# qiyueyao/Kubernetes-verification

Hardware: AMD Instinct MI355X
Metric: pod-pairs/sec for reachability build + all-checks latency, 100k pods, 1/2/4/8 GPU (higher is better)
Workload: dtype u64

## Files before the change

### include/kano_hip.h

```cpp
#ifndef KANO_HIP_H
#define KANO_HIP_H

#include <stddef.h>
#include <stdint.h>

#ifdef __cplusplus
extern "C" {
#endif

typedef struct kano_ctx kano_ctx;

#define KANO_PATH_AUTO    0
#define KANO_PATH_BITWISE 1
#define KANO_PATH_MFMA    2

#define KANO_INFO_N        0
#define KANO_INFO_W        1
#define KANO_INFO_P        2
#define KANO_INFO_U        3
#define KANO_INFO_NNZ_SEL  4
#define KANO_INFO_NNZ_ALW  5
#define KANO_INFO_HEAVY    6
#define KANO_INFO_ROW0     7
#define KANO_INFO_ROW1     8
#define KANO_INFO_MAXSEL   9
#define KANO_INFO_UA      10
#define KANO_INFO_HEAVY_PATH 11
#define KANO_INFO_WORK_ITEMS 12
#define KANO_INFO_ROWS_KERNEL 13
#define KANO_INFO_ROWS_CUS 14
#define KANO_INFO_HEAVY_SEL 15
#define KANO_INFO_HEAVY_KERNEL 16
#define KANO_INFO_CLS_REUSED 17
#define KANO_INFO_NSLOTS   18

int  kano_create(int device, kano_ctx** out);
int  kano_create_lean(int device, kano_ctx** out);
void kano_destroy(kano_ctx* ctx);
const char* kano_last_error(const kano_ctx* ctx);
int  kano_set_stream(kano_ctx* ctx, void* hip_stream);

int kano_set_pods(kano_ctx* ctx, int64_t n, int32_t ncols, const int32_t* pod_val);
int kano_set_policies(kano_ctx* ctx, int64_t P,
                      const int64_t* sel_off, const int32_t* sel_col, const int32_t* sel_val,
                      const int64_t* alw_off, const int32_t* alw_col, const int32_t* alw_val);
int kano_set_shard(kano_ctx* ctx, int64_t row_begin, int64_t row_end);

int kano_build(kano_ctx* ctx, int path);
int kano_info(kano_ctx* ctx, int64_t* out );

int kano_col_checks(kano_ctx* ctx, uint64_t* col_and, uint64_t* col_or);
int kano_col_flags_dev(kano_ctx* ctx, uint8_t* flags_dev);

int kano_crosscheck(kano_ctx* ctx, const int32_t* gid, uint64_t* cross);
int kano_crosscheck_dev(kano_ctx* ctx, const int32_t* gid, uint8_t* flags_dev);

int kano_get_rows(kano_ctx* ctx, int64_t r0, int64_t nrows, uint64_t* dst);
// ... 205 lines not shown
```

### kubernetes-verification_amd/csrc/kano_engine.hpp

```cpp
#pragma once
#include <hip/hip_runtime.h>
#include <hip/hip_ext.h>

#include <algorithm>
#include <cmath>
#include <functional>
#include <cerrno>
#include <cstdint>
#include <cstdlib>
#include <cstring>
#include <string>
#include <vector>
#include <array>
#include <chrono>
#include <ctime>
#include <cstdio>
#include <dlfcn.h>
#include <link.h>
#include <thread>

#include "kano_hip.h"
#include "kano_internal.hpp"
#include "kano_pairwalk.hpp"
#include "kano_prims.hpp"
// ... 115 lines not shown
  int group_grid = 0;
  int group_batches = 0;
  int shadow_r = 0;
  int shg_sub_lds = 1;
  int rows_cu_off = 20;
  int xcd_split = 1;
  i64 xcd_min_bytes = XCD_MIN_BYTES;
  int xcd_write = XCD_WRITE;
  int xcd_eng0 = -1;
  bool xcd_tried = false, eng_on_xcd = false, xcd_last_ok = false;
  int side_mode = 0;
  int xcd_side = -1;
  hipStream_t stream_x = nullptr, stream2_x = nullptr, stream3x = nullptr;
  hipStream_t stream2_u = nullptr;
  hipEvent_t ev_sw = nullptr, ev_sw2 = nullptr;
  i64 rows_cu_bytes = 8ll << 30;
  int num_cus = 0, rows_cus = 0;

  ClassSet rc, cc;
  bool cls_valid = false;
  bool cls_reuse = false;
  i64 cls_U[2] = {0, 0};
  i64 cls_reused = 0;
  SideMatch sm, am;
  i64 UAW = 0, ldC = 0;
  i64 nnz_sel = 0, nnz_alc = 0, nnz_alw = 0, heavy_count = 0, wi_total = 0, nflags = 0;
  i64 heavy_sel = 0;
  i64 light_cost = 0;
  bool rows_use_alist = false;
  int max_sel = 0;
  int heavy_path = 0;
  int heavy_kernel = 0;
  int rows_kernel = 0;

  DBuf pv;
  DBuf scnt, cost, soffc, scur, slist, ecls, wicls, maxs, wicnt, wioff, hflag, hoff, hlist, sq, pfoff;
  DBuf ACT, AC, nca, acnt, alcoff, alc, aloff, alist;
  DBuf M, Mc, color, colnand, col_and, col_or_c, col_nand_c;
  DBuf scan_tmp;
  i64 scan_cap = 0;
  int scan_parity = 0;
  DBuf scan_tmp2;
  i64 scan_cap2 = 0;
  int scan_parity2 = 0;
  hipEvent_t ev_pre = nullptr, ev_pre_done = nullptr, ev_pre_ac = nullptr;
  bool pre_forked = false, pre_side_pending = false, pre_ac_pending = false;
// ... 202 lines not shown
```

### kubernetes-verification_amd/csrc/kano_hip.hip

```cpp
#include "kano_engine.hpp"
#include "kano_kernels.hpp"

namespace kano_eng {

int fail(kano_ctx* ctx, int code, const std::string& msg) {
  ctx->err = msg;
  return code;
}

int settle(kano_ctx* ctx);

int dalloc(kano_ctx* ctx, DBuf& b, size_t bytes) {
  if (bytes == 0) bytes = 16;
  if (b.p && b.bytes >= bytes) return 0;
  if (b.p) {
    KTRY(settle(ctx));
    KCHK(hipFree(b.p));
    b.p = nullptr;
    b.bytes = 0;
  }
  const hipError_t e = hipMalloc(&b.p, bytes);
  if (e != hipSuccess) {
    b.p = nullptr;
    return fail(ctx, -ENOMEM, "hipMalloc(" + std::to_string(bytes) + " bytes) -> " +
// ... 1062 lines not shown
  if (ctx->pre_side_pending) {
    ctx->pre_side_pending = false;
    KTRY(join_event(ctx, ctx->ev_pre_done));
  }
  ctx->alist_valid = false;
  ctx->rows_use_alist = ctx->light_cost > 0 && ctx->light_cost * 16 > ctx->nnz_alw &&
                        ctx->nnz_alw * 4 <= (2ll << 30);
  const McScatterArgs msa{ctx->nnz_sel, P_<int32_t>(ctx->ecls), P_<int32_t>(ctx->slist),
                          P_<i64>(ctx->alcoff), P_<int32_t>(ctx->alc), P_<int32_t>(ctx->rc.mcnt),
                          H > 0 ? P_<int32_t>(ctx->hflag) : (const int32_t*)nullptr,
                          P_<u64>(ctx->Mc), ldMc};
  const bool scatter_on = U > 0 && ctx->nnz_sel > 0;
  const bool pods_in_scatter = ctx->rows_use_alist && scatter_on && P > 0 && ctx->cc.U > 0;
  if (ctx->rows_use_alist) KTRY(build_alist(ctx, nullptr, !pods_in_scatter));
  ctx->rin_marked = false;
  if (U == 0) return ctx->fork_hook ? ctx->fork_hook(fork_marked) : 0;
  hipEvent_t rin_mark = H == 0 && ctx->cols_deferred ? ctx->ev_rin_e : nullptr;
  if (scatter_on && (size_t)ldMc * 8 * (TPB / 64) <= 64 * 1024) {
    const size_t lds = sizeof(u64) * (size_t)ldMc * (TPB / 64);
    const McOwnArgs moa{U, P_<i64>(ctx->soffc), P_<int32_t>(ctx->slist), P_<i64>(ctx->alcoff),
                        P_<int32_t>(ctx->alc), P_<int32_t>(ctx->rc.mcnt),
                        H > 0 ? P_<int32_t>(ctx->hflag) : (const int32_t*)nullptr,
                        P_<u64>(ctx->Mc), ldMc};
    if (pods_in_scatter) {
      const unsigned nb1 = nblk(P, WPB);
      hipExtLaunchKernelGGL(k_pods_own, dim3(nb1 + nblk(U, TPB / 64)), dim3(TPB), lds,
                            ctx->stream, nullptr, rin_mark, 0, pol_pods_args(ctx), moa, nb1);
    } else {
      hipExtLaunchKernelGGL(k_mc_own, dim3(nblk(U, TPB / 64)), dim3(TPB), lds, ctx->stream,
                            nullptr, rin_mark, 0, moa);
    }
    KLAUNCH();
    ctx->rin_marked = rin_mark != nullptr;
  } else if (scatter_on) {
    if (pods_in_scatter) {
      const unsigned nb1 = nblk(P, WPB);
      hipExtLaunchKernelGGL(k_pods_scatter, dim3(nb1 + nblk(ctx->nnz_sel, TPB / 64)), dim3(TPB),
                            0, ctx->stream, nullptr, rin_mark, 0, pol_pods_args(ctx), msa, nb1);
    } else {
      hipExtLaunchKernelGGL(k_mc_scatter, dim3(nblk(ctx->nnz_sel, TPB / 64)), dim3(TPB), 0,
                            ctx->stream, nullptr, rin_mark, 0, msa);
    }
    KLAUNCH();
    ctx->rin_marked = rin_mark != nullptr;
  }
  if (H > 0) {
    if (mfma) {
// ... 82 lines not shown
    } else {
      if (ctx->time_or) {
        KTRY(resolve_mfma_time(ctx));
        KCHK(hipEventRecord(ctx->ev_m0, ctx->stream));
      }
      hipLaunchKernelGGL(k_heavy_mc_or, dim3((unsigned)H, nblk(ldMc, 64)), dim3(TPB), 0, ctx->stream,
                         P_<int32_t>(ctx->hlist), P_<i64>(ctx->soffc), P_<int32_t>(ctx->slist),
                         P_<u64>(ctx->AC), ctx->ldC, ctx->UAW, P_<u64>(ctx->Mc), ldMc);
      KLAUNCH();
      if (ctx->time_or) {
        KCHK(hipEventRecord(ctx->ev_m1, ctx->stream));
        ctx->mfma_time_pending = true;
        ctx->mfma_ops_last = 2.0 * (double)H * (double)P * (double)ctx->cc.U;
      }
    }
    const bool early = ctx->rows_early_heavy == 1 ||
                       (ctx->rows_early_heavy == 2 &&
                        std::min<i64>(ctx->ldM, ctx->rows_cww) > 4096);
    if (early && ctx->cols_deferred && !ctx->rin_marked) {
      KCHK(hipEventRecord(ctx->ev_rin_e, ctx->stream));
      ctx->rin_marked = true;
    }
  }
  if (!ctx->cols_deferred) KTRY(mc_cols(ctx));
  if (ctx->fork_hook) KTRY(ctx->fork_hook(fork_marked));
  return 0;
}

int do_rows(kano_ctx* ctx) {
  const i64 ldM = ctx->ldM, n = ctx->n;
  if (n > 0) {
    hipLaunchKernelGGL(k_cols_expand, dim3(nblk(ldM * 64)), dim3(TPB), 0, ctx->stream,
                       P_<u64>(ctx->col_or_c), P_<u64>(ctx->col_nand_c), P_<int32_t>(ctx->cc.cls),
                       n, ldM, P_<u64>(ctx->color), P_<u64>(ctx->colnand));
    KLAUNCH();
  } else {
    KCHK(hipMemsetAsync(ctx->color.p, 0, sizeof(u64) * ldM, ctx->stream));
    KCHK(hipMemsetAsync(ctx->colnand.p, 0, sizeof(u64) * ldM, ctx->stream));
  }
  return 0;
}

thread_local bool g_create_lean = false;
void rows_cu_mask(int K, uint32_t* mask) {
  const int t = K < 4 ? 1 : K / 4, beta = K < 4 ? K : 4;
  for (int w = 0; w < 8; ++w) {
    mask[w] = 0xffffffffu;
// ... 296 lines not shown
  int32_t G = ngroups;
  cp.gdev = P_<int32_t>(ctx->gid);
  if (!gid) {
    if (ctx->groups_n != n) return fail(ctx, -EINVAL, "crosscheck: no stored groups for these pods");
    G = ctx->groups_G;
    cp.gdev = P_<int32_t>(ctx->gids);
  } else {
    if (G <= 0) {
      G = 0;
      for (i64 i = 0; i < n; ++i) {
        if (gid[i] < 0) return fail(ctx, -EINVAL, "kano_crosscheck: negative group id");
        G = std::max(G, gid[i] + 1);
      }
    }
    KCHK(hipMemcpyAsync(ctx->gid.p, gid, sizeof(int32_t) * n, hipMemcpyHostToDevice,
                        st ? st : ctx->stream));
  }
  cp.G = G;
  cp.on = true;
  return 0;
}

int cross_prepare(kano_ctx* ctx, const int32_t* gid, int32_t ngroups, CrossPlan& cp,
                  FillBatch& fb, bool setup_done = false) {
  const i64 ldM = ctx->ldM;
  if (!setup_done) KTRY(cross_setup(ctx, gid, ngroups, cp, fb.st));
  int32_t* err = reinterpret_cast<int32_t*>(P_<u64>(ctx->sizes) + SZ_ERR);
  KTRY(fb.add_raw(err, sizeof(u64), 0u));
  KTRY(fb.add(ctx->cross, sizeof(u64) * ldM, 0u));
  if (!cp.on) return 0;
  const int32_t G = cp.G;
  if (ctx->rows_dirty) return 0;
  const i64 U = ctx->rc.U, ldC = ctx->ldC;
  KTRY(dalloc(ctx, ctx->gmin, sizeof(int32_t) * std::max<i64>(1, U)));
  KTRY(dalloc(ctx, ctx->gmax, sizeof(int32_t) * std::max<i64>(1, U)));
  KTRY(dalloc(ctx, ctx->R, sizeof(u64) * std::max<i64>(1, (i64)G * ldC)));
  KTRY(dalloc(ctx, ctx->ckey, sizeof(int32_t) * std::max<i64>(1, U)));
  KTRY(dalloc(ctx, ctx->corder, sizeof(int32_t) * std::max<i64>(1, U)));
  cp.key_lds = (i64)G + 1 <= KEY_LDS_MAX;
  cp.knb = std::max<i64>(1, nblk(U, (i64)TPB * KEY_ITEMS));
  cp.kslots = cp.key_lds ? ((i64)G + 1) * cp.knb : (i64)G + 1;
  KTRY(dalloc(ctx, ctx->kcnt, sizeof(int32_t) * 2 * ((i64)G + 1) + sizeof(int32_t) * cp.kslots));
  KTRY(dalloc(ctx, ctx->koff, sizeof(int32_t) * (cp.kslots + 1)));
  KTRY(dalloc(ctx, ctx->multi, sizeof(u64) * ldC));
  KTRY(dalloc(ctx, ctx->A1, sizeof(u64) * ldC));
  KTRY(dalloc(ctx, ctx->A2, sizeof(u64) * ldC));
  KTRY(fb.add(ctx->gmin, sizeof(int32_t) * U, 0x7fffffffu));
  KTRY(fb.add(ctx->gmax, sizeof(int32_t) * U, 0xffffffffu));
  KTRY(fb.add(ctx->R, sizeof(u64) * (i64)G * ldC, 0u));
  for (DBuf* b : {&ctx->multi, &ctx->A1, &ctx->A2}) KTRY(fb.add(*b, sizeof(u64) * ldC, 0u));
  KTRY(fb.add(ctx->kcnt, sizeof(int32_t) * 2 * ((i64)G + 1), 0u));
  return 0;
}

KeySort cross_sort(kano_ctx* ctx, const CrossPlan& cp) {
  KeySort k{};
  k.U = ctx->rc.U;
  k.nb = cp.knb;
  k.mcnt = P_<int32_t>(ctx->rc.mcnt);
  k.gmin = P_<int32_t>(ctx->gmin);
  k.gmax = P_<int32_t>(ctx->gmax);
  k.G = cp.G;
  k.ckey = P_<int32_t>(ctx->ckey);
  k.hist = P_<int32_t>(ctx->kcnt) + 2 * ((i64)cp.G + 1);
  k.hoff = P_<int32_t>(ctx->koff);
  k.order = P_<int32_t>(ctx->corder);
  return k;
}

int cross_stage_a(kano_ctx* ctx, const CrossPlan& cp, ScanBatch& sb, hipStream_t st = nullptr) {
  if (!cp.on) return 0;
  const i64 U = ctx->rc.U, G = cp.G, rl = rows_local(ctx);
  const hipStream_t s = st ? st : ctx->stream;
  int32_t* err = reinterpret_cast<int32_t*>(P_<u64>(ctx->sizes) + SZ_ERR);
  hipLaunchKernelGGL(k_cls_group_range_m, dim3(nblk(rl)), dim3(TPB), 0, s, cp.gdev,
                     (int32_t)G, P_<int32_t>(ctx->rc.cls), P_<int32_t>(ctx->rc.mem), rl,
                     P_<int32_t>(ctx->gmin), P_<int32_t>(ctx->gmax), err);
  KLAUNCH();
  int32_t* kcnt = P_<int32_t>(ctx->kcnt);
  if (cp.key_lds) {
    const KeySort ks = cross_sort(ctx, cp);
    hipLaunchKernelGGL(k_key_hist, dim3((unsigned)cp.knb), dim3(TPB),
                       sizeof(int32_t) * (size_t)(G + 1), s, ks);
    KLAUNCH();
    if (!st) KTRY(sb.add(ks.hist, cp.kslots, P_<int32_t>(ctx->koff)));
  } else {
    hipLaunchKernelGGL(k_cls_key, dim3(nblk(U)), dim3(TPB), 0, s, U,
                       P_<int32_t>(ctx->rc.mcnt), P_<int32_t>(ctx->gmin), P_<int32_t>(ctx->gmax),
                       (int32_t)G, P_<int32_t>(ctx->ckey), kcnt);
    KLAUNCH();
    KTRY(sb.add(kcnt, G + 1, P_<int32_t>(ctx->koff)));
  }
  return 0;
}

int cross_stage_b1(kano_ctx* ctx, const CrossPlan& cp, hipStream_t st = nullptr) {
  if (!cp.on) return 0;
  const i64 U = ctx->rc.U, G = cp.G;
  const hipStream_t s = st ? st : ctx->stream;
  int32_t* kcnt = P_<int32_t>(ctx->kcnt);
  if (cp.key_lds && st) {
    hipLaunchKernelGGL(k_key_place_scan, dim3((unsigned)cp.knb), dim3(TPB),
                       sizeof(int32_t) * (size_t)(G + 1), s, cross_sort(ctx, cp));
  } else if (cp.key_lds) {
    hipLaunchKernelGGL(k_key_place_lds, dim3((unsigned)cp.knb), dim3(TPB),
                       sizeof(int32_t) * (size_t)(G + 1), s, cross_sort(ctx, cp));
  } else {
    hipLaunchKernelGGL(k_cls_key_place, dim3(nblk(U)), dim3(TPB), 0, s, U,
                       P_<int32_t>(ctx->ckey), P_<int32_t>(ctx->koff), kcnt + G + 1,
                       P_<int32_t>(ctx->corder));
  }
  KLAUNCH();
  return 0;
}

int cross_stage_b2(kano_ctx* ctx, const CrossPlan& cp) {
  if (!cp.on) return 0;
  const i64 U = ctx->rc.U, G = cp.G, ldC = ctx->ldC, UAW = ctx->UAW;
  const bool cols = ctx->cols_deferred;
  const int32_t* nlive = P_<int32_t>(ctx->koff) + cp.kslots;
  {
    const int32_t* ord = P_<int32_t>(ctx->corder);
    const int32_t* ck = P_<int32_t>(ctx->ckey);
    u64* co = cols ? P_<u64>(ctx->col_or_c) : nullptr;
    u64* cn = cols ? P_<u64>(ctx->col_nand_c) : nullptr;
    const dim3 g(nblk(UAW, 64), nblk(U, (TPB / 64) * FOLD_PER_WAVE));
    hipLaunchKernelGGL(k_mc_fold, g, dim3(TPB), 0, ctx->stream, P_<u64>(ctx->Mc), ldC, UAW,
                       ctx->cc.U, ord, nlive, ck, (int32_t)G, P_<u64>(ctx->R),
                       P_<u64>(ctx->multi), co, cn);
  }
  KLAUNCH();
  ctx->cols_deferred = false;
  hipLaunchKernelGGL(k_cross_groups, dim3((unsigned)G, nblk(UAW)), dim3(TPB), 0, ctx->stream,
                     P_<u64>(ctx->R), ldC, UAW, P_<u64>(ctx->A1), P_<u64>(ctx->A2));
  KLAUNCH();
  ctx->cross_G = (int32_t)G;
  return 0;
}

int crosscheck_impl(kano_ctx* ctx, const int32_t* gid, int32_t ngroups = 0) {
  const i64 n = ctx->n, W = ctx->W, ldM = ctx->ldM;
  CrossPlan cp;
  {
    FillBatch fb(ctx);
// ... 276 lines not shown
        if (k == "pmf" && v >= 0 && v <= 2) ctx->pmask_form = v;
        if (k == "pmgrid" && v >= 0) ctx->pmask_grid = v;
        if (k == "pvf" && v >= 0 && v <= 2) ctx->verdict_form = v;
        if (k == "pvgrid" && v >= 0) ctx->verdict_grid = v;
        if (k == "dgrid" && v >= 0) ctx->diff_grid = v;
        if (k == "ggrid" && v >= 0) ctx->group_grid = v;
        if (k == "gbatch" && v >= 0) ctx->group_batches = v;
        if (k == "shr" && (v == 1 || v == 2 || v == 4 || v == 8)) ctx->shadow_r = v;
        if (k == "rcu" && v >= 0 && v <= 28 && (v < 4 || v % 4 == 0)) ctx->rows_cu_off = v;
        if (k == "rcubytes" && v >= 0) ctx->rows_cu_bytes = (i64)v << 30;
        if (k == "xcd") ctx->xcd_split = v;
        if (k == "xcdmin" && v >= 0) ctx->xcd_min_bytes = (i64)v << 10;
        if (k == "xcdw" && v >= 1 && v <= 7) ctx->xcd_write = v;
        if (k == "xcde" && v >= 0 && v <= 7) ctx->xcd_eng0 = v;
        if (k == "xcdside" && v >= -1 && v <= 1) ctx->xcd_side = v;
        if (k == "hgemm" && (v == -1 || v == 0 || v == 22 || v == 42 || v == 44))
          ctx->heavy_gemm = v;
        if (k == "hgemmmin" && v > 0) ctx->heavy_gemm_min = v;
        if (k == "hortime") ctx->time_or = v;
        if (k == "hexplds" && v >= 2 && v <= 4) ctx->heavy_expand_lds = v;
        if (k == "dx") ctx->dx_on = v;
        if (k == "aclds") ctx->ac_lds = v;
        if (k == "mlside") ctx->mlists_side_ok = v;
        if (k == "xomfma" && v > 0) ctx->xo_mfma = (double)v * 1e12;
        if (k == "xoor" && v > 0) ctx->xo_or = (double)v * 1e9;
      }
      pos = end + 1;
    }
  }
  int prio_lo = 0, prio_hi = 0;
  (void)hipDeviceGetStreamPriorityRange(&prio_lo, &prio_hi);
  (void)prio_lo;

  const int prio_main = prio_hi;
  if (hipStreamCreateWithPriority(&ctx->stream, hipStreamNonBlocking, prio_main) != hipSuccess) {
    delete ctx;
    return -EIO;
  }
  ctx->own_stream = true;
  mark("stream");
  for (auto& e : ctx->ev) (void)hipEventCreate(&e);
  mark("stage_events");
  {
    const int lds44 = (int)(sizeof(u64) * 2 * GK_KC * (256 + 256));
    (void)hipFuncSetAttribute(reinterpret_cast<const void*>(&k_heavy_gemm_f4<4, 4, gemm_kc(4, 4)>),
                              hipFuncAttributeMaxDynamicSharedMemorySize, lds44);
// ... 453 lines not shown
    return 0;
  }
  hipLaunchKernelGGL(k_sel_place, dim3(nblk(P, sel_spb(ctx))), dim3(TPB), 0, ctx->stream, P,
                     P_<i64>(ctx->sm.pstart), P_<int32_t>(ctx->sm.plen), P_<int32_t>(ctx->sm.gmem),
                     P_<i64>(ctx->soffc), P_<int32_t>(ctx->scur), P_<int32_t>(ctx->slist),
                     P_<int32_t>(ctx->ecls), sel_spb(ctx), FillJobs{}, nblk(P, sel_spb(ctx)), cap);
  KLAUNCH();
  ctx->sel_early_cap = cap;
  return 0;
}

int build_impl(kano_ctx* ctx, int path, bool rows_now, bool defer_cols = false,
               const ExtraFills& extra = ExtraFills(), const ExtraFills& pre_fill = ExtraFills(),
               const PreRun& pre_run = PreRun()) {
  if (!ctx) return -EINVAL;
  const bool consume = ctx->primed && ctx->consume_prime;
  ctx->consume_prime = false;
  if (!consume) KTRY(unprime(ctx));
  if (!ctx->have_pods || !ctx->have_pols) return fail(ctx, -EINVAL, "kano_build: inputs not set");
  if (path < 0 || path > 2) return fail(ctx, -EINVAL, "kano_build: unknown path");
  KCHK(hipSetDevice(ctx->device));
  ctx->cls_reuse = consume ? ctx->prime_kept : ctx->cls_valid;
  ctx->cls_valid = false;
  ctx->built = false;
  ctx->rows_deferred = false;
  ctx->lists_mode = false;
  ctx->rows_timed = false;
  ctx->rows_dirty = false;
  ctx->cols_valid = false;
  ctx->shadow_total = -1;
  ctx->conflict_total = -1;
  ctx->sig_armed = 0;
  ctx->sel_early_cap = -1;
  ctx->shg_prefilled = false;
  const i64 rl = rows_local(ctx);
  if (!ctx->defer_alloc)
    KTRY(dalloc(ctx, ctx->M, sizeof(u64) * std::max<i64>(1, rl * ctx->ldM)));
  KTRY(dalloc(ctx, ctx->color, sizeof(u64) * ctx->ldM));
  KTRY(dalloc(ctx, ctx->colnand, sizeof(u64) * ctx->ldM));
  KTRY(stage_mark(ctx, 0, ctx->stream));
  KTRY(do_front(ctx, path, consume));
  KTRY(mirror_begin(ctx));
  KTRY(do_back_pre(ctx, pre_fill, pre_run));
  KTRY(sel_place_early(ctx));
  KTRY(read_sizes(ctx));
  KTRY(stage_mark(ctx, 3, ctx->stream));
// ... 30 lines not shown
}

int kano_info(kano_ctx* ctx, int64_t* out) {
  if (!ctx || !out) return -EINVAL;
  for (int k = 0; k < KANO_INFO_NSLOTS; ++k) out[k] = 0;
  out[KANO_INFO_N] = ctx->n;
  out[KANO_INFO_W] = ctx->W;
  out[KANO_INFO_P] = ctx->P;
  out[KANO_INFO_U] = ctx->rc.U;
  out[KANO_INFO_NNZ_SEL] = ctx->nnz_sel;
  out[KANO_INFO_NNZ_ALW] = ctx->nnz_alw;
  out[KANO_INFO_HEAVY] = ctx->heavy_count;
  out[KANO_INFO_ROW0] = ctx->r0;
  out[KANO_INFO_ROW1] = ctx->r1;
  out[KANO_INFO_MAXSEL] = ctx->max_sel;
  out[KANO_INFO_UA] = ctx->cc.U;
  out[KANO_INFO_HEAVY_PATH] = ctx->heavy_path;
  out[KANO_INFO_ROWS_CUS] = ctx->rows_cus;
  out[KANO_INFO_HEAVY_SEL] = ctx->heavy_sel;
  out[KANO_INFO_HEAVY_KERNEL] = ctx->heavy_kernel;
  out[KANO_INFO_WORK_ITEMS] = ctx->wi_total;
  out[KANO_INFO_ROWS_KERNEL] = ctx->rows_kernel;
  out[KANO_INFO_CLS_REUSED] = ctx->cls_reused;
  return 0;
}

int kano_col_checks(kano_ctx* ctx, uint64_t* col_and, uint64_t* col_or) {
  KTRY(ensure_matrix(ctx));
  if (!ctx->cols_valid) KTRY(recompute_cols(ctx));
  const i64 W = ctx->W;
  if (W == 0) return sync(ctx);
  KTRY(dalloc(ctx, ctx->col_and, sizeof(u64) * W));
  hipLaunchKernelGGL(k_col_final, dim3(nblk(W)), dim3(TPB), 0, ctx->stream,
                     P_<u64>(ctx->colnand), W, ctx->n, P_<u64>(ctx->col_and));
  KLAUNCH();
  if (col_and)
    KCHK(hipMemcpyAsync(col_and, ctx->col_and.p, sizeof(u64) * W, hipMemcpyDeviceToHost,
                        ctx->stream));
  if (col_or)
    KCHK(hipMemcpyAsync(col_or, ctx->color.p, sizeof(u64) * W, hipMemcpyDeviceToHost, ctx->stream));
  return sync(ctx);
}

int kano_col_flags_dev(kano_ctx* ctx, uint8_t* flags_dev) {
  KTRY(ensure_matrix(ctx));
  if (!ctx->cols_valid) KTRY(recompute_cols(ctx));
// ... 1032 lines not shown
      if (void* h = dlopen(path.c_str(), RTLD_NOW | RTLD_NOLOAD)) f = dlsym(h, "ncclAllGather");
    }
    if (!f) f = dlsym(RTLD_DEFAULT, "ncclAllGather");
    if (!f) {
      void* h = dlopen("librccl.so", RTLD_NOW | RTLD_GLOBAL);
      if (!h) h = dlopen("librccl.so.1", RTLD_NOW | RTLD_GLOBAL);
      if (h) f = dlsym(h, "ncclAllGather");
    }
    return reinterpret_cast<RcclAllGather>(f);
  }();
  return fn;
}

int verify_front(kano_ctx* ctx, int path, const int32_t* gid, int32_t ngroups, int64_t sys_row,
                 bool want_shadow, u64* words_dev, bool count_only = false) {
  ctx->vs_count_only = want_shadow && count_only;
  ctx->consume_prime = ctx->primed;
  if (ctx->async_pending && !ctx->primed) KTRY(swap_rows_inputs(ctx));
  const bool stored = !gid && ngroups == KANO_STORED_GROUPS;
  const bool want_cross = gid || stored;
  CrossPlan cp;
  ShadowPlan sp;
  auto pre_fill = [&](FillBatch& fb) -> int {
    return want_cross ? cross_prepare(ctx, gid, ngroups, cp, fb) : 0;
  };
  auto pre_run = [&](hipStream_t st) -> int {
    if (!want_cross || !cp.on) return 0;
    ScanBatch sb(ctx, st != nullptr);
    KTRY(cross_stage_a(ctx, cp, sb, st));
    KTRY(sb.run());
    return cross_stage_b1(ctx, cp, st);
  };
  auto extra = [&](FillBatch& fb) -> int {
    return want_shadow ? shadow_prepare(ctx, sp, fb) : 0;
  };
  ctx->vs_open = false;
  ctx->fork_pending = false;
  ctx->tail_compacted = false;
  bool fork_marked = false;
  const bool side_sh = want_shadow && !count_only;
  if (want_shadow) {
    ctx->fork_hook = [&](bool marked) -> int {
      if (!marked) KCHK(hipEventRecord(ctx->ev_fork2, ctx->stream));
      KCHK(hipStreamWaitEvent(ctx->stream2, ctx->ev_fork2, 0));
      KTRY(shadow_test_launch(ctx, sp, ctx->stream2));
      fork_marked = true;
      return 0;
    };
  }
  const int brc = build_impl(ctx, path, false, want_cross, extra, pre_fill, pre_run);
  ctx->fork_hook = nullptr;
  KTRY(brc);
  const i64 n = ctx->n, W = ctx->W;
  const bool have_sys = sys_row >= ctx->r0 && sys_row < ctx->r1;
  const bool cross_on = want_cross && cp.on;
  if (cross_on) KTRY(cross_stage_b2(ctx, cp));
  const bool side_run = fork_marked && side_sh;
  if (!side_run && fork_marked) {
    KCHK(hipEventRecord(ctx->ev_join2, ctx->stream2));
    ctx->fork_pending = true;
  }
  if (want_shadow && !side_run) {
    ScanBatch sb(ctx);
    if (ctx->fork_pending) {
      KCHK(hipStreamWaitEvent(ctx->stream, ctx->ev_join2, 0));
      ctx->fork_pending = false;
      KTRY(shadow_stage_a_scans(ctx, sp, sb));
    } else {
      KTRY(shadow_stage_a(ctx, sp, sb));
    }
    KTRY(sb.run());
  }
  if (ctx->cols_deferred) {
    ctx->cols_deferred = false;
    KTRY(mc_cols(ctx));
  }
  const i64 nb = std::max<i64>(1, nblk(W * 64));
  KTRY(dalloc(ctx, ctx->col_and, sizeof(u64) * std::max<i64>(1, W)));
  KTRY(dalloc(ctx, ctx->sysrow, sizeof(u64) * std::max<i64>(1, W)));
// ... 52 lines not shown
                                P_<i64>(ctx->poff), SZ_PAIRS));
      KTRY(sbs.run(sp.nt > 0 ? nullptr : ctx->ev_pairs));
    }
    KTRY(dalloc(ctx, ctx->L, sizeof(int2) * std::max<i64>(1, sp.nf)));
    if (sp.nt > 0) {
      launch_marked(k_shadow_compact, dim3((unsigned)sp.nt), dim3(TPB), 0, s2, ctx->ev_pairs,
                    P_<i64>(ctx->soffc), ctx->rc.U, P_<int32_t>(ctx->slist),
                    P_<i64>(ctx->pfoff), P_<uint8_t>(ctx->flags), sp.nf, P_<i64>(ctx->toff),
                    P_<int2>(ctx->L), sp.nf);
      KLAUNCH();
    }
    ctx->tail_compacted = true;
  }
  ctx->vs_open = true;
  ctx->vs_shadow = want_shadow;
  ctx->vs_cross_want = want_cross;
  ctx->vs_cross_on = cross_on;
  ctx->vs_have_sys = have_sys;
  ctx->vs_sys_on = sys_on;
  ctx->vs_rows = true;
  ctx->vs_nb = nb;
  ctx->vs_rl = sp.rl;
  return 0;
}

int spin_event(kano_ctx* ctx, hipEvent_t e) {
  using clk = std::chrono::steady_clock;
  const auto t0 = clk::now();
  for (uint32_t spin = 1;; ++spin) {
    const hipError_t q = hipEventQuery(e);
    if (q == hipSuccess) return 0;
    if (q != hipErrorNotReady) KCHK(q);
    __builtin_ia32_pause();
    if ((spin & 0xff) == 0 && clk::now() - t0 > std::chrono::seconds(1)) {
      KCHK(hipEventSynchronize(e));
      return 0;
    }
  }
}

int prime_next(kano_ctx* ctx) {
  if (ctx->primed || !ctx->bell || ctx->stage_timing) return 0;
  KTRY(dalloc(ctx, ctx->sizes_alt, sizeof(u64) * SZ_SLOTS));
  ctx->prime_alist_valid = ctx->alist_valid;
  ctx->prime_kept = ctx->cls_valid;
  ctx->cls_reuse = ctx->cls_valid;
// ... 76 lines not shown
                          0, cj);
    KLAUNCH();
  }
  if (ctx->vs_rows) {
    ctx->rows_overlap = async;
    ctx->rows_in = ctx->rin_marked ? ctx->ev_rin_e : ctx->ev_tail;
    ctx->rin_marked = false;
    const int rc = launch_rows(ctx);
    ctx->rows_overlap = false;
    ctx->rows_in = nullptr;
    KTRY(rc);
  }
  if (async && ctx->pipeline) KTRY(prime_next(ctx));
  part(12);
  const auto tw0 = clk::now();
  KTRY(spin_event(ctx, ctx->ev_tail));
  ctx->ht[18] += std::chrono::duration<double, std::micro>(clk::now() - tw0).count();
  part(14);
  ctx->sig_wait = 0;
  constexpr int NS = SZ_ERR - SZ_NL + 1;
  i64 v[NS];
  for (int q = 0; q < NS; ++q) v[q] = (i64)((volatile u64*)ctx->gmirror)[SZ_NL + q];
  if (ctx->vs_cross_on && (v[SZ_ERR - SZ_NL] & 0xffffffff)) {
    (void)settle(ctx);
    (void)sync(ctx);
    return fail(ctx, -EINVAL, "kano_verify: a group id lies outside [0, ngroups)");
  }
  for (int r = 0; r < 4; ++r) counts[r] = v[SZ_IDX0 - SZ_NL + r];
  if (!ctx->vs_have_sys) counts[3] = -1;
  if (want_shadow) {
    const i64 total = v[SZ_PAIRS - SZ_NL];
    *shadow_count = total;
    ctx->shadow_total = pairs_mode ? total : -1;
    if (pairs_mode && total > out_cap) {
      KTRY(unprime(ctx));
      KTRY(dalloc(ctx, ctx->out, sizeof(int2) * (total + total / 4)));
      if (rl > 0) {
        hipLaunchKernelGGL(k_shadow_emit, dim3(nblk(rl)), dim3(TPB), 0, st,
                           P_<int32_t>(ctx->rc.cls), ctx->r0, ctx->r1, P_<i64>(ctx->loff),
                           P_<int2>(ctx->L), P_<i64>(ctx->poff), P_<int2>(ctx->out), total,
                           (const i64*)nullptr, nf);
        KLAUNCH();
      }
      if (shadow_pairs && total <= shadow_cap)
        KTRY(copy_out(ctx, shadow_pairs, ctx->out.p, sizeof(int2) * total, st));
      KCHK(hipEventRecord(ctx->ev_tail, st));
      KCHK(hipEventSynchronize(ctx->ev_tail));
    }
  }
  part(15);
// ... 64 lines not shown
    return verify_back_direct(ctx, idx, idx_h, counts, shadow_pairs, pairs_h, shadow_cap,
                              shadow_count, may_async && ctx->async_rows, compacted);
  constexpr int NS = SZ_ERR - SZ_NL + 1;
  using clk = std::chrono::steady_clock;
  auto tmark = clk::now();
  auto part = [&](int k) {
    const auto t = clk::now();
    ctx->ht[k] = std::max(ctx->ht[k], std::chrono::duration<double, std::micro>(t - tmark).count());
    tmark = t;
  };
  const bool signalled = ctx->sig_armed != 0;
  KTRY(mirror_begin(ctx));
  hipEvent_t tail_ev = signalled ? nullptr : ctx->ev_sizes;
  const bool async = may_async && ctx->async_rows;
  if (!tail_ev) {
    KCHK(hipEventRecord(ctx->ev_sizes, ctx->stream));
    tail_ev = ctx->ev_sizes;
  }
  part(12);
  i64 v[NS];
  KTRY(mirror_wait(ctx, SZ_NL, NS, v));
  tmark = clk::now();
  if (ctx->vs_cross_on && (v[SZ_ERR - SZ_NL] & 0xffffffff)) {
    (void)sync(ctx);
    return fail(ctx, -EINVAL, "kano_verify: a group id lies outside [0, ngroups)");
  }
  i64 nidx = 0;
  for (int r = 0; r < 4; ++r) {
    counts[r] = v[SZ_IDX0 - SZ_NL + r];
    nidx += counts[r];
  }
  if (!ctx->vs_have_sys) counts[3] = -1;
  hipStream_t cs = ctx->stream2;
  KCHK(hipStreamWaitEvent(cs, tail_ev, 0));
  i64 total = 0;
  if (want_shadow) {
    total = v[SZ_PAIRS - SZ_NL];
    if (shadow_cap >= 0) {
      KTRY(shadow_back(ctx, v[0], total, cs));
      part(13);
      ctx->shadow_total = total;
    } else {
      ctx->shadow_total = -1;
    }
    *shadow_count = total;
  }
  tmark = clk::now();
  if (nidx > 0) {
    KTRY(copy_out(ctx, idx, idx_dev, sizeof(int32_t) * nidx, cs));
// ... 230 lines not shown
}

int kano_set_groups(kano_ctx* ctx, const int32_t* gid, int32_t ngroups) {
  if (!ctx) return -EINVAL;
  if (!ctx->have_pods) return fail(ctx, -EINVAL, "kano_set_groups before kano_set_pods");
  const i64 n = ctx->n;
  if (n > 0 && !gid) return fail(ctx, -EINVAL, "kano_set_groups: gid is NULL");
  KCHK(hipSetDevice(ctx->device));
  KTRY(settle(ctx));
  int32_t G = 0;
  for (i64 i = 0; i < n; ++i) {
    if (gid[i] < 0) return fail(ctx, -EINVAL, "kano_set_groups: negative group id");
    G = std::max(G, gid[i] + 1);
  }
  if (ngroups > 0 && ngroups < G) return fail(ctx, -EINVAL, "kano_set_groups: id >= ngroups");
  if (ngroups > 0) G = ngroups;
  KTRY(dalloc(ctx, ctx->gids, sizeof(int32_t) * std::max<i64>(1, n)));
  if (n > 0)
    KCHK(hipMemcpyAsync(ctx->gids.p, gid, sizeof(int32_t) * n, hipMemcpyHostToDevice,
                        ctx->stream));
  KTRY(sync(ctx));
  ctx->groups_n = n;
  ctx->groups_G = G;
  return 0;
}

int kano_host_alloc(size_t bytes, void** out) {
  if (!out) return -EINVAL;
  *out = nullptr;
  if (hipHostMalloc(out, bytes ? bytes : 16, hipHostMallocDefault) != hipSuccess) return -ENOMEM;
  return 0;
}

void kano_host_free(void* p) {
  if (p) (void)hipHostFree(p);
}

int kano_stage_times(kano_ctx* ctx, float* ms) {
  if (!ctx || !ms) return -EINVAL;
  KCHK(hipSetDevice(ctx->device));
  KTRY(settle(ctx));
  KTRY(sync(ctx));
  for (int k = 0; k < 8; ++k) ms[k] = 0.f;
  if (ctx->built && !ctx->lists_mode) {
    if (ctx->stage_timing) {
      for (int k = 0; k < 4; ++k) (void)hipEventElapsedTime(&ms[k], ctx->ev[k], ctx->ev[k + 1]);
// ... 83 lines not shown
```

### kubernetes-verification_amd/csrc/kano_kernels.hpp

```cpp
#pragma once
#include "kano_pairwalk.hpp"
#include "kano_prims.hpp"

namespace kano {

struct ClsSide {
  const int32_t* keys;
  int KS;
  int packed;
  int pbits;
  uint32_t tmask;
  int32_t* table;
  int32_t* slot_of;
  int32_t* smin;
  int32_t* flag;
  const int32_t* cid;
  int32_t* cls;
  int32_t* rep;
  int32_t* mcnt;
  int32_t* mcur;
  const int32_t* moff;
  int32_t* mem;
  int32_t* cval;
  i64 m0, m1, U;
// ... 1159 lines not shown
  }
  __builtin_amdgcn_fence(__ATOMIC_ACQ_REL, "workgroup");
  __builtin_amdgcn_wave_barrier();
  u64* dst = a.Mc + c * a.ldMc;
  for (i64 w = lane; w < a.ldMc; w += 64) {
    const u64 v = row[w];
    if (v) dst[w] = v;
  }
}
__global__ __launch_bounds__(TPB) void k_mc_own(McOwnArgs a) {
  extern __shared__ __attribute__((aligned(16))) u64 mrow[];
  mc_own_item(a, blockIdx.x, mrow);
}

__global__ __launch_bounds__(TPB) void k_pods_scatter(PolPodsArgs a, McScatterArgs b,
                                                      unsigned nb1) {
  if (blockIdx.x < nb1) pol_pods_item(a, blockIdx.x);
  else mc_scatter_item(b, blockIdx.x - nb1);
}
__global__ __launch_bounds__(TPB) void k_pods_own(PolPodsArgs a, McOwnArgs b, unsigned nb1) {
  extern __shared__ __attribute__((aligned(16))) u64 mrow[];
  if (blockIdx.x < nb1) pol_pods_item(a, blockIdx.x);
  else mc_own_item(b, blockIdx.x - nb1, mrow);
}


__global__ __launch_bounds__(TPB) void k_mc_cols(const u64* __restrict__ Mc, i64 ldMc, i64 UW,
                                                 i64 Ua, i64 U, const int32_t* __restrict__ mcnt,
                                                 u64* col_or_c, u64* col_nand_c) {
  __shared__ u64 red[2][4][64];
  const int lane = threadIdx.x & 63, wid = threadIdx.x >> 6;
  const i64 w = (i64)blockIdx.x * 64 + lane;
  const i64 c0 = (i64)blockIdx.y * 128 + wid * 32;
  const u64 vm = w < UW ? valid_mask(w, Ua) : 0ull;
  u64 o = 0, na = 0;
  if (w < UW) {
    for (i64 c = c0; c < min(c0 + 32, U); ++c) {
      if (mcnt[c] == 0) continue;
      const u64 v = Mc[c * ldMc + w];
      o |= v;
      na |= ~v & vm;
    }
  }
  red[0][wid][lane] = o;
  red[1][wid][lane] = na;
  __syncthreads();
// ... 2387 lines not shown
```

### kubernetes-verification_amd/kano/_native.py

```python
from __future__ import annotations

import ctypes
import os
from ctypes import POINTER, c_double, c_float, c_int, c_int32, c_int64, c_uint8, c_uint64, c_void_p

_HERE = os.path.dirname(os.path.abspath(__file__))
LIB_PATH = os.environ.get(
    "KANO_HIP_LIB", os.path.join(os.path.dirname(_HERE), "csrc", "libkano_hip.so"))

SIGNATURES = {
    "kano_create": (c_int, [c_int, POINTER(c_void_p)]),
    "kano_create_lean": (c_int, [c_int, POINTER(c_void_p)]),
    "kano_destroy": (None, [c_void_p]),
    "kano_last_error": (ctypes.c_char_p, [c_void_p]),
    "kano_set_stream": (c_int, [c_void_p, c_void_p]),
    "kano_set_pods": (c_int, [c_void_p, c_int64, c_int32, c_void_p]),
    "kano_set_policies": (c_int, [c_void_p, c_int64, c_void_p, c_void_p, c_void_p,
                                  c_void_p, c_void_p, c_void_p]),
    "kano_set_shard": (c_int, [c_void_p, c_int64, c_int64]),
    "kano_build": (c_int, [c_void_p, c_int]),
    "kano_info": (c_int, [c_void_p, c_void_p]),
    "kano_col_checks": (c_int, [c_void_p, c_void_p, c_void_p]),
    "kano_col_flags_dev": (c_int, [c_void_p, c_void_p]),
    "kano_crosscheck": (c_int, [c_void_p, c_void_p, c_void_p]),
# ... 92 lines not shown
    "kano_group_create_lean": (c_int, [c_int, c_void_p, POINTER(c_void_p)]),
    "kano_group_create_ex": (c_int, [c_int, c_void_p, c_int, POINTER(c_void_p)]),
    "kano_group_destroy": (None, [c_void_p]),
    "kano_group_last_error": (ctypes.c_char_p, [c_void_p]),
    "kano_group_info": (c_int, [c_void_p, c_void_p]),
    "kano_group_member": (c_int, [c_void_p, c_int, POINTER(c_void_p)]),
    "kano_group_verify": (c_int, [c_void_p, c_int, c_void_p, c_int32, c_int64, c_int, c_void_p,
                                  c_void_p, c_void_p, c_int64, POINTER(c_int64)]),
    "kano_group_checks": (c_int, [c_void_p, c_void_p, c_int32, c_int64, c_void_p, c_void_p]),
    "kano_group_upload": (c_int, [c_void_p, c_int64, c_int32, c_void_p, c_int32, c_void_p,
                                  c_void_p, c_void_p, c_void_p, c_int64, c_void_p, c_void_p,
                                  c_void_p, c_void_p, c_void_p, c_void_p, c_void_p]),
    "kano_group_build": (c_int, [c_void_p, c_int]),
    "kano_group_set_groups": (c_int, [c_void_p, c_void_p, c_int32]),
    "kano_group_add_policies": (c_int, [c_void_p, c_int64, c_int32, c_void_p] + [c_void_p] * 6 +
                                [POINTER(c_int64)]),
    "kano_group_remove_policies": (c_int, [c_void_p, c_int64, c_void_p]),
    "kano_group_path": (c_int, [c_void_p, c_void_p, c_int, c_int, c_void_p]),
    "kano_group_exchange_timing": (c_int, [c_void_p, c_int, c_void_p, c_int]),
    "kano_host_alloc": (c_int, [ctypes.c_size_t, POINTER(c_void_p)]),
    "kano_host_free": (None, [c_void_p]),
}

INFO_SLOTS = 18
INFO = dict(N=0, W=1, P=2, U=3, NNZ_SEL=4, NNZ_ALW=5, HEAVY=6, ROW0=7, ROW1=8, MAXSEL=9,
            UA=10, HEAVY_PATH=11, WORK_ITEMS=12, ROWS_KERNEL=13, ROWS_CUS=14,
            HEAVY_SEL=15, HEAVY_KERNEL=16, CLS_REUSED=17)
PATHS = {"auto": 0, "bitwise": 1, "mfma": 2}
STORED_GROUPS = -1
GROUP_LEAN, GROUP_RCCL, GROUP_COPY = 1, 2, 4


class KanoNativeError(RuntimeError):
    pass


_lib = None


def load(path: str = LIB_PATH) -> ctypes.CDLL:
    global _lib
    if _lib is not None:
        return _lib
    if not os.path.exists(path):
        raise KanoNativeError(
            f"{path} not found: build it with `python -c 'import __graft_entry__ as g; g.build()'`")
    lib = ctypes.CDLL(path)
    for name, (res, args) in SIGNATURES.items():
        fn = getattr(lib, name)
        fn.restype = res
# ... 26 lines not shown
```

Before: 32950 billion.

## Reuse cross-check group ordering across builds and add fused own-scatter fold kernel

When groups are stored and the pod classes are reused from the previous build, the cross-check ordering (gmin/gmax, key counts, scans) is kept. Stages A and B1 are skipped, and only the R/multi/A buffers are re-zeroed. A generation counter and commit-on-success logic invalidate the kept ordering when groups change or a verify fails. A new opt-in kernel fuses the Mc owner scatter with the per-group OR fold and the column OR/NAND reduction, which removes a separate pass over Mc. It adds LDS use and atomics, and its correctness relies on the ordering being contiguous per key.

```diff
diff --git a/include/kano_hip.h b/include/kano_hip.h
--- a/include/kano_hip.h
+++ b/include/kano_hip.h
@@ -32,7 +32,9 @@
 #define KANO_INFO_HEAVY_SEL 15
 #define KANO_INFO_HEAVY_KERNEL 16
 #define KANO_INFO_CLS_REUSED 17
-#define KANO_INFO_NSLOTS   18
+#define KANO_INFO_ORD_REUSED 18
+#define KANO_INFO_OWN_FOLDED 19
+#define KANO_INFO_NSLOTS   20
 
 int  kano_create(int device, kano_ctx** out);
 int  kano_create_lean(int device, kano_ctx** out);
diff --git a/kubernetes-verification_amd/csrc/kano_engine.hpp b/kubernetes-verification_amd/csrc/kano_engine.hpp
--- a/kubernetes-verification_amd/csrc/kano_engine.hpp
+++ b/kubernetes-verification_amd/csrc/kano_engine.hpp
@@ -161,6 +161,20 @@
   bool cls_reuse = false;
   i64 cls_U[2] = {0, 0};
   i64 cls_reused = 0;
+  bool ord_valid = false;
+  bool ord_reuse = false;
+  bool ord_cand = false;
+  u64 groups_gen = 0;
+  u64 ord_gen = 0;
+  int32_t ord_G = 0;
+  i64 ord_U = 0, ord_kslots = 0, ord_r0 = 0, ord_r1 = 0;
+  i64 ord_reused = 0;
+  i64 own_folded = 0;
+  int cross_keep = 1;
+  int own_fold = 0;
+  bool fold_ok = false, fold_fused = false;
+  int32_t fold_G = 0;
+  i64 fold_kslots = 0;
   SideMatch sm, am;
   i64 UAW = 0, ldC = 0;
   i64 nnz_sel = 0, nnz_alc = 0, nnz_alw = 0, heavy_count = 0, wi_total = 0, nflags = 0;
diff --git a/kubernetes-verification_amd/csrc/kano_hip.hip b/kubernetes-verification_amd/csrc/kano_hip.hip
--- a/kubernetes-verification_amd/csrc/kano_hip.hip
+++ b/kubernetes-verification_amd/csrc/kano_hip.hip
@@ -1108,7 +1108,21 @@
                         P_<int32_t>(ctx->alc), P_<int32_t>(ctx->rc.mcnt),
                         H > 0 ? P_<int32_t>(ctx->hflag) : (const int32_t*)nullptr,
                         P_<u64>(ctx->Mc), ldMc};
-    if (pods_in_scatter) {
+    ctx->fold_fused = ctx->fold_ok && ctx->own_fold && H == 0 && ctx->cols_deferred &&
+                      ldMc <= OWNFOLD_MAX_LD;
+    if (ctx->fold_fused) {
+      const unsigned nb1 = pods_in_scatter ? nblk(P, WPB) : 0u;
+      const size_t flds = sizeof(u64) * (size_t)ldMc * ((TPB / 64) * OWNFOLD_SUB + 3);
+      const McFoldArgs mfa{P_<int32_t>(ctx->corder), P_<int32_t>(ctx->koff) + ctx->fold_kslots,
+                           P_<int32_t>(ctx->ckey), ctx->fold_G, ctx->UAW, ctx->cc.U,
+                           P_<u64>(ctx->R), P_<u64>(ctx->multi), P_<u64>(ctx->col_or_c),
+                           P_<u64>(ctx->col_nand_c)};
+      hipExtLaunchKernelGGL(k_pods_own_fold,
+                            dim3(nb1 + nblk(U, (TPB / 64) * OWNFOLD_PER_WAVE)), dim3(TPB), flds,
+                            ctx->stream, nullptr, rin_mark, 0, pol_pods_args(ctx), moa, mfa, nb1);
+      ctx->cols_deferred = false;
+      ++ctx->own_folded;
+    } else if (pods_in_scatter) {
       const unsigned nb1 = nblk(P, WPB);
       hipExtLaunchKernelGGL(k_pods_own, dim3(nb1 + nblk(U, TPB / 64)), dim3(TPB), lds,
                             ctx->stream, nullptr, rin_mark, 0, pol_pods_args(ctx), moa, nb1);
@@ -1237,7 +1251,7 @@
       ctx->rin_marked = true;
     }
   }
-  if (!ctx->cols_deferred) KTRY(mc_cols(ctx));
+  if (!ctx->cols_deferred && !ctx->fold_fused) KTRY(mc_cols(ctx));
   if (ctx->fork_hook) KTRY(ctx->fork_hook(fork_marked));
   return 0;
 }
@@ -1580,8 +1594,10 @@
 }
 
 int cross_prepare(kano_ctx* ctx, const int32_t* gid, int32_t ngroups, CrossPlan& cp,
-                  FillBatch& fb, bool setup_done = false) {
+                  FillBatch& fb, bool setup_done = false, bool may_keep = false) {
   const i64 ldM = ctx->ldM;
+  ctx->ord_reuse = false;
+  ctx->ord_cand = false;
   if (!setup_done) KTRY(cross_setup(ctx, gid, ngroups, cp, fb.st));
   int32_t* err = reinterpret_cast<int32_t*>(P_<u64>(ctx->sizes) + SZ_ERR);
   KTRY(fb.add_raw(err, sizeof(u64), 0u));
@@ -1603,10 +1619,16 @@
   KTRY(dalloc(ctx, ctx->multi, sizeof(u64) * ldC));
   KTRY(dalloc(ctx, ctx->A1, sizeof(u64) * ldC));
   KTRY(dalloc(ctx, ctx->A2, sizeof(u64) * ldC));
+  ctx->ord_reuse = may_keep && !gid && ctx->cross_keep && ctx->ord_valid && ctx->cls_reuse &&
+                   ctx->ord_gen == ctx->groups_gen && ctx->ord_G == G && ctx->ord_U == U &&
+                   ctx->ord_kslots == cp.kslots && ctx->ord_r0 == ctx->r0 &&
+                   ctx->ord_r1 == ctx->r1;
+  KTRY(fb.add(ctx->R, sizeof(u64) * (i64)G * ldC, 0u));
+  for (DBuf* b : {&ctx->multi, &ctx->A1, &ctx->A2}) KTRY(fb.add(*b, sizeof(u64) * ldC, 0u));
+  if (ctx->ord_reuse) return 0;
+  ctx->ord_valid = false;
   KTRY(fb.add(ctx->gmin, sizeof(int32_t) * U, 0x7fffffffu));
   KTRY(fb.add(ctx->gmax, sizeof(int32_t) * U, 0xffffffffu));
-  KTRY(fb.add(ctx->R, sizeof(u64) * (i64)G * ldC, 0u));
-  for (DBuf* b : {&ctx->multi, &ctx->A1, &ctx->A2}) KTRY(fb.add(*b, sizeof(u64) * ldC, 0u));
   KTRY(fb.add(ctx->kcnt, sizeof(int32_t) * 2 * ((i64)G + 1), 0u));
   return 0;
 }
@@ -1627,7 +1649,7 @@
 }
 
 int cross_stage_a(kano_ctx* ctx, const CrossPlan& cp, ScanBatch& sb, hipStream_t st = nullptr) {
-  if (!cp.on) return 0;
+  if (!cp.on || ctx->ord_reuse) return 0;
   const i64 U = ctx->rc.U, G = cp.G, rl = rows_local(ctx);
   const hipStream_t s = st ? st : ctx->stream;
   int32_t* err = reinterpret_cast<int32_t*>(P_<u64>(ctx->sizes) + SZ_ERR);
@@ -1653,7 +1675,7 @@
 }
 
 int cross_stage_b1(kano_ctx* ctx, const CrossPlan& cp, hipStream_t st = nullptr) {
-  if (!cp.on) return 0;
+  if (!cp.on || ctx->ord_reuse) return 0;
   const i64 U = ctx->rc.U, G = cp.G;
   const hipStream_t s = st ? st : ctx->stream;
   int32_t* kcnt = P_<int32_t>(ctx->kcnt);
@@ -1677,7 +1699,9 @@
   const i64 U = ctx->rc.U, G = cp.G, ldC = ctx->ldC, UAW = ctx->UAW;
   const bool cols = ctx->cols_deferred;
   const int32_t* nlive = P_<int32_t>(ctx->koff) + cp.kslots;
-  {
+  if (ctx->fold_fused) {
+    ctx->fold_fused = false;
+  } else {
     const int32_t* ord = P_<int32_t>(ctx->corder);
     const int32_t* ck = P_<int32_t>(ctx->ckey);
     u64* co = cols ? P_<u64>(ctx->col_or_c) : nullptr;
@@ -2000,6 +2024,8 @@
         if (k == "dx") ctx->dx_on = v;
         if (k == "aclds") ctx->ac_lds = v;
         if (k == "mlside") ctx->mlists_side_ok = v;
+        if (k == "crosskeep") ctx->cross_keep = v;
+        if (k == "ownfold") ctx->own_fold = v;
         if (k == "xomfma" && v > 0) ctx->xo_mfma = (double)v * 1e12;
         if (k == "xoor" && v > 0) ctx->xo_or = (double)v * 1e9;
       }
@@ -2499,6 +2525,10 @@
   KCHK(hipSetDevice(ctx->device));
   ctx->cls_reuse = consume ? ctx->prime_kept : ctx->cls_valid;
   ctx->cls_valid = false;
+  if (!ctx->cls_reuse) ctx->ord_valid = false;
+  ctx->ord_reuse = false;
+  ctx->ord_cand = false;
+  ctx->fold_ok = ctx->fold_fused = false;
   ctx->built = false;
   ctx->rows_deferred = false;
   ctx->lists_mode = false;
@@ -2575,6 +2605,8 @@
   out[KANO_INFO_WORK_ITEMS] = ctx->wi_total;
   out[KANO_INFO_ROWS_KERNEL] = ctx->rows_kernel;
   out[KANO_INFO_CLS_REUSED] = ctx->cls_reused;
+  out[KANO_INFO_ORD_REUSED] = ctx->ord_reused;
+  out[KANO_INFO_OWN_FOLDED] = ctx->own_folded;
   return 0;
 }
 
@@ -3653,7 +3685,12 @@
   CrossPlan cp;
   ShadowPlan sp;
   auto pre_fill = [&](FillBatch& fb) -> int {
-    return want_cross ? cross_prepare(ctx, gid, ngroups, cp, fb) : 0;
+    if (!want_cross) return 0;
+    KTRY(cross_prepare(ctx, gid, ngroups, cp, fb, false, stored));
+    ctx->fold_ok = cp.on && (!gid || ngroups <= 0);
+    ctx->fold_G = cp.G;
+    ctx->fold_kslots = cp.kslots;
+    return 0;
   };
   auto pre_run = [&](hipStream_t st) -> int {
     if (!want_cross || !cp.on) return 0;
@@ -3686,6 +3723,17 @@
   const bool have_sys = sys_row >= ctx->r0 && sys_row < ctx->r1;
   const bool cross_on = want_cross && cp.on;
   if (cross_on) KTRY(cross_stage_b2(ctx, cp));
+  if (cross_on && stored && ctx->cross_keep) {
+    if (ctx->ord_reuse) ++ctx->ord_reused;
+    ctx->ord_gen = ctx->groups_gen;
+    ctx->ord_G = cp.G;
+    ctx->ord_U = ctx->rc.U;
+    ctx->ord_kslots = cp.kslots;
+    ctx->ord_r0 = ctx->r0;
+    ctx->ord_r1 = ctx->r1;
+    ctx->ord_cand = true;
+  }
+  ctx->ord_reuse = false;
   const bool side_run = fork_marked && side_sh;
   if (!side_run && fork_marked) {
     KCHK(hipEventRecord(ctx->ev_join2, ctx->stream2));
@@ -3784,6 +3832,11 @@
   ctx->vs_nb = nb;
   ctx->vs_rl = sp.rl;
   return 0;
+}
+
+void ord_commit(kano_ctx* ctx) {
+  if (ctx->ord_cand) ctx->ord_valid = true;
+  ctx->ord_cand = false;
 }
 
 int spin_event(kano_ctx* ctx, hipEvent_t e) {
@@ -3906,10 +3959,12 @@
   i64 v[NS];
   for (int q = 0; q < NS; ++q) v[q] = (i64)((volatile u64*)ctx->gmirror)[SZ_NL + q];
   if (ctx->vs_cross_on && (v[SZ_ERR - SZ_NL] & 0xffffffff)) {
+    ctx->ord_valid = ctx->ord_cand = false;
     (void)settle(ctx);
     (void)sync(ctx);
     return fail(ctx, -EINVAL, "kano_verify: a group id lies outside [0, ngroups)");
   }
+  ord_commit(ctx);
   for (int r = 0; r < 4; ++r) counts[r] = v[SZ_IDX0 - SZ_NL + r];
   if (!ctx->vs_have_sys) counts[3] = -1;
   if (want_shadow) {
@@ -4020,9 +4075,11 @@
   KTRY(mirror_wait(ctx, SZ_NL, NS, v));
   tmark = clk::now();
   if (ctx->vs_cross_on && (v[SZ_ERR - SZ_NL] & 0xffffffff)) {
+    ctx->ord_valid = ctx->ord_cand = false;
     (void)sync(ctx);
     return fail(ctx, -EINVAL, "kano_verify: a group id lies outside [0, ngroups)");
   }
+  ord_commit(ctx);
   i64 nidx = 0;
   for (int r = 0; r < 4; ++r) {
     counts[r] = v[SZ_IDX0 - SZ_NL + r];
@@ -4299,6 +4356,7 @@
   KTRY(sync(ctx));
   ctx->groups_n = n;
   ctx->groups_G = G;
+  ++ctx->groups_gen;
   return 0;
 }
 
diff --git a/kubernetes-verification_amd/csrc/kano_kernels.hpp b/kubernetes-verification_amd/csrc/kano_kernels.hpp
--- a/kubernetes-verification_amd/csrc/kano_kernels.hpp
+++ b/kubernetes-verification_amd/csrc/kano_kernels.hpp
@@ -1205,6 +1205,142 @@
   extern __shared__ __attribute__((aligned(16))) u64 mrow[];
   if (blockIdx.x < nb1) pol_pods_item(a, blockIdx.x);
   else mc_own_item(b, blockIdx.x - nb1, mrow);
+}
+
+constexpr int OWNFOLD_PER_WAVE = 2;
+constexpr int OWNFOLD_SUB = 2;
+constexpr int OWNFOLD_WPL = 8;
+constexpr int OWNFOLD_MAX_LD = 64 * OWNFOLD_WPL;
+struct McFoldArgs {
+  const int32_t* order;
+  const int32_t* nlive;
+  const int32_t* ckey;
+  int32_t G;
+  i64 UW, Ua;
+  u64* R;
+  u64* multi;
+  u64* col_or;
+  u64* col_nand;
+};
+__device__ __forceinline__ i64 shfl_i64(i64 v, int src) {
+  const int lo = __shfl((int)(v & 0xffffffffll), src, 64), hi = __shfl((int)(v >> 32), src, 64);
+  return ((i64)hi << 32) | (i64)(uint32_t)lo;
+}
+__device__ __forceinline__ void mc_own_fold_item(const McOwnArgs& a, const McFoldArgs& f, i64 vb,
+                                                 u64* lds) {
+  constexpr int NW = TPB / 64, PW = OWNFOLD_PER_WAVE, SUB = OWNFOLD_SUB, WPL = OWNFOLD_WPL;
+  constexpr int SL = 64 / SUB;
+  const int lane = threadIdx.x & 63, wv = threadIdx.x >> 6;
+  const i64 ld = a.ldMc;
+  const i64 nlive = *f.nlive;
+  const i64 kb = vb * (NW * PW);
+  if (kb >= nlive) return;
+  u64* rows = lds + (i64)wv * SUB * ld;
+  u64* bo = lds + (i64)NW * SUB * ld;
+  u64* bna = bo + ld;
+  u64* bacc = bna + ld;
+  for (i64 w = threadIdx.x; w < 3 * ld; w += TPB) bo[w] = 0;
+  const int32_t kfirst = f.ckey[f.order[kb]];
+  __syncthreads();
+  const i64 k0 = kb + (i64)wv * PW;
+  const int cnt = (int)max((i64)0, min(nlive, k0 + PW) - k0);
+  int32_t myc = 0, myk = -1;
+  i64 mye0 = 0, mye1 = 0;
+  if (lane < cnt) {
+    myc = f.order[k0 + lane];
+    myk = f.ckey[myc];
+    mye0 = a.soffc[myc];
+    mye1 = a.soffc[myc + 1];
+  }
+  u64 o[WPL], na[WPL], acc[WPL], vm[WPL];
+#pragma unroll
+  for (int j = 0; j < WPL; ++j) {
+    const i64 w = lane + 64 * j;
+    o[j] = na[j] = acc[j] = 0;
+    vm[j] = w < f.UW ? valid_mask(w, f.Ua) : 0ull;
+  }
+  int32_t cur = -1;
+  auto flush = [&]() {
+    if (cur < 0) return;
+    u64* d = cur == f.G ? f.multi : f.R + (i64)cur * ld;
+#pragma unroll
+    for (int j = 0; j < WPL; ++j) {
+      const i64 w = lane + 64 * j;
+      if (acc[j]) {
+        if (cur == kfirst) atomicOr(&bacc[w], acc[j]);
+        else if (acc[j] & ~d[w]) atomicOr(&d[w], acc[j]);
+      }
+      acc[j] = 0;
+    }
+  };
+  const int sub = lane / SL, sl = lane % SL;
+  for (int q0 = 0; q0 < cnt; q0 += SUB) {
+    for (i64 w = lane; w < SUB * ld; w += 64) rows[w] = 0;
+    __builtin_amdgcn_fence(__ATOMIC_RELEASE, "workgroup");
+    __builtin_amdgcn_wave_barrier();
+    {
+      const int q = q0 + sub;
+      const i64 e0 = shfl_i64(mye0, q & 63), e1 = shfl_i64(mye1, q & 63);
+      u64* row = rows + (i64)sub * ld;
+      if (q < cnt) {
+        for (i64 e = e0 + sl; e < e1; e += SL) {
+          const int32_t p = a.slist[e];
+          const i64 q1 = a.alcoff[p + 1];
+          for (i64 t = a.alcoff[p]; t < q1; ++t) {
+            const int32_t ca = a.alc[t];
+            atomicOr(&row[ca >> 6], 1ull << (ca & 63));
+          }
+        }
+      }
+    }
+    __builtin_amdgcn_fence(__ATOMIC_ACQ_REL, "workgroup");
+    __builtin_amdgcn_wave_barrier();
+    for (int s = 0; s < SUB && q0 + s < cnt; ++s) {
+      const int q = q0 + s;
+      const int32_t c = __shfl(myc, q, 64), key = __shfl(myk, q, 64);
+      const bool empty = shfl_i64(mye0, q) == shfl_i64(mye1, q);
+      if (key != cur) {
+        flush();
+        cur = key;
+      }
+      const u64* row = rows + (i64)s * ld;
+      u64* dst = a.Mc + (i64)c * ld;
+#pragma unroll
+      for (int j = 0; j < WPL; ++j) {
+        const i64 w = lane + 64 * j;
+        u64 v = 0;
+        if (!empty && w < ld) {
+          v = row[w];
+          if (v) dst[w] = v;
+        }
+        o[j] |= v;
+        acc[j] |= v;
+        na[j] |= ~v & vm[j];
+      }
+    }
+    __builtin_amdgcn_wave_barrier();
+  }
+  flush();
+#pragma unroll
+  for (int j = 0; j < WPL; ++j) {
+    const i64 w = lane + 64 * j;
+    if (o[j]) atomicOr(&bo[w], o[j]);
+    if (na[j]) atomicOr(&bna[w], na[j]);
+  }
+  __syncthreads();
+  u64* d = kfirst == f.G ? f.multi : f.R + (i64)kfirst * ld;
+  for (i64 w = threadIdx.x; w < f.UW; w += TPB) {
+    const u64 vo = bo[w], vn = bna[w], va = bacc[w];
+    if (vo & ~f.col_or[w]) atomicOr(&f.col_or[w], vo);
+    if (vn & ~f.col_nand[w]) atomicOr(&f.col_nand[w], vn);
+    if (va & ~d[w]) atomicOr(&d[w], va);
+  }
+}
+__global__ __launch_bounds__(TPB) void k_pods_own_fold(PolPodsArgs a, McOwnArgs b, McFoldArgs f,
+                                                       unsigned nb1) {
+  extern __shared__ __attribute__((aligned(16))) u64 mrow[];
+  if (blockIdx.x < nb1) pol_pods_item(a, blockIdx.x);
+  else mc_own_fold_item(b, f, blockIdx.x - nb1, mrow);
 }
 
 
diff --git a/kubernetes-verification_amd/kano/_native.py b/kubernetes-verification_amd/kano/_native.py
--- a/kubernetes-verification_amd/kano/_native.py
+++ b/kubernetes-verification_amd/kano/_native.py
@@ -138,10 +138,10 @@
     "kano_host_free": (None, [c_void_p]),
 }
 
-INFO_SLOTS = 18
+INFO_SLOTS = 20
 INFO = dict(N=0, W=1, P=2, U=3, NNZ_SEL=4, NNZ_ALW=5, HEAVY=6, ROW0=7, ROW1=8, MAXSEL=9,
             UA=10, HEAVY_PATH=11, WORK_ITEMS=12, ROWS_KERNEL=13, ROWS_CUS=14,
-            HEAVY_SEL=15, HEAVY_KERNEL=16, CLS_REUSED=17)
+            HEAVY_SEL=15, HEAVY_KERNEL=16, CLS_REUSED=17, ORD_REUSED=18, OWN_FOLDED=19)
 PATHS = {"auto": 0, "bitwise": 1, "mfma": 2}
 STORED_GROUPS = -1
 GROUP_LEAN, GROUP_RCCL, GROUP_COPY = 1, 2, 4
```

New measurement: 32600 billion. -1.1%, worse.
